# Kloudy-Sky/openintel

Measured on AMD Instinct MI355X. Metric: queries/sec + p50 latency, 10M-post/768-d hybrid BM25+cosine+RRF top-100, higher is better.
Workload: dtype f32

## Files before the change

### openintel_amd/csrc/select.hip

```cpp
#include "oi_device.h"
#include "oi_internal.h"

#define SEL_THREADS 1024
#define SEL_MAX 1024

__device__ void bitonic_sort_desc(uint64_t *a, uint32_t P) {
    const uint32_t tid = threadIdx.x;
    for (uint32_t size = 2; size <= P; size <<= 1) {
        for (uint32_t stride = size >> 1; stride > 0; stride >>= 1) {
            for (uint32_t t = tid; t < (P >> 1); t += SEL_THREADS) {
                uint32_t lo = 2 * t - (t & (stride - 1));
                uint32_t hi = lo + stride;
                bool desc = ((lo & size) == 0);
                uint64_t x = a[lo], y = a[hi];
                if ((x < y) == desc) { a[lo] = y; a[hi] = x; }
            }
            __syncthreads();
        }
    }
}

#define SEL_LDS_KEYS 8192

struct SelSource {
// ... 82 lines not shown
            if (tid < 64) {
                const uint32_t kk = s_kk;
                uint32_t mine = 0;
                for (int i = 0; i < 4; ++i) mine += hist[255 - (tid * 4 + i)];
                uint32_t incl = mine;
#pragma unroll
                for (int o = 1; o < 64; o <<= 1) {
                    uint32_t v = __shfl_up(incl, o, OI_WAVE);
                    if ((int)tid >= o) incl += v;
                }
                const unsigned long long ball = __ballot(incl >= kk);
                const uint32_t owner = ball ? (uint32_t)__builtin_ctzll(ball) : 63u;
                if (tid == owner) {
                    uint32_t cum = incl - mine;
                    int d = 255 - (int)(tid * 4);
                    for (int i = 0; i < 3; ++i, --d) {
                        const uint32_t c = hist[d];
                        if (cum + c >= kk) break;
                        cum += c;
                    }
                    s_prefix = (prefix << 8) | (uint64_t)d;
                    s_kk = kk - cum;
                    s_bin_cnt = hist[d];
                }
            }
            __syncthreads();
            if (s_bin_cnt == 1 || shift == 0) break;
        }
        const uint64_t prefix = s_prefix;
        sel_for_each(S, [&](uint64_t key) {
            if ((key >> shift) >= prefix) {
                const uint32_t pos = atomicAdd(&s_cnt, 1u);
                if (pos < SEL_MAX) sel[pos] = key;
            }
        });
        __syncthreads();
        m = s_cnt < k ? s_cnt : k;
    }
    __shared__ unsigned long long s_min;
    if (out_scores) {
        uint32_t P = 2;
        while (P < m) P <<= 1;
        for (uint32_t i = m + tid; i < P; i += SEL_THREADS) sel[i] = 0;
        __syncthreads();
        bitonic_sort_desc(sel, P);
        for (uint32_t i = tid; i < m; i += SEL_THREADS) {
            const uint64_t key = sel[i];
            out_scores[(uint64_t)q * out_stride + i] = oi_rank_key_score(key);
            out_docs[(uint64_t)q * out_stride + i] = oi_rank_key_doc(key);
        }
        if (tid == 0) { out_counts[q] = m; s_min = m ? sel[m - 1] : 0; }
    } else {
        if (tid == 0) s_min = ~0ull;
        __syncthreads();
        unsigned long long lo = ~0ull;
        for (uint32_t i = tid; i < m; i += SEL_THREADS) lo = sel[i] < lo ? sel[i] : lo;
#pragma unroll
        for (int o = 32; o > 0; o >>= 1) {
            const unsigned long long v = __shfl_xor(lo, o, OI_WAVE);
            lo = v < lo ? v : lo;
        }
        if ((tid & 63) == 0 && lo != ~0ull) atomicMin(&s_min, lo);
    }
    __syncthreads();
    if (compact) {
        for (uint32_t i = tid; i < m; i += SEL_THREADS) pool[i] = sel[i];
        for (uint32_t sg = tid; sg < n_segs; sg += SEL_THREADS) segc[sg] = 0;
        if (tid == 0) {
            carry_cnt[q] = m;
            if (m == k && tau_keys) {
                const uint32_t t = (uint32_t)(s_min >> 32);
                if (t > tau_keys[q]) tau_keys[q] = t;
            }
        }
    }
}

#define SEL_MAX_SEGS 4096
#define SEL_KPT_MAX 32
#ifdef OI_ABLATION
__device__ int sel_dbg_on;
__device__ unsigned long long sel_dbg_t[16];
#define SEL_STAMP(i) do { if (sel_dbg_on && blockIdx.x == 0 && threadIdx.x == 0) sel_dbg_t[i] = __builtin_readcyclecounter(); } while (0)
#else
#define SEL_STAMP(i) do { } while (0)
#endif
#define SEL_CAND 4096

struct SelRowMargin {
    const float *meta;
    uint32_t base;
    float qn, cq;
};
__device__ __forceinline__ float sel_row_e(const SelRowMargin *rm, uint64_t kv) {
    return rm->meta[2 * (uint64_t)(oi_rank_key_doc(kv) - rm->base) + 1];
}
__device__ __forceinline__ bool sel_row_test(const SelRowMargin *rm, uint64_t kv, float e, float edge, float eps2) {
    const float u = oi_rank_key_score(kv) + 2.002f * (e * rm->qn + rm->cq);
    return u >= edge - 9.5367431640625e-07f * (fabsf(edge) + eps2);
}
__device__ __forceinline__ bool sel_row_keep(const SelRowMargin *rm, uint64_t kv, float edge, float eps2) {
    if (!rm) return true;
    return sel_row_test(rm, kv, sel_row_e(rm, kv), edge, eps2);
}

__device__ __forceinline__ void sel_spec_words(bool have, uint32_t rth_key, float eps2, uint32_t tau, uint32_t *spec_tau, uint32_t *spec_max) {
    if (!have) { *spec_tau = tau; return; }
    const float s = oi_key_f32(rth_key) - eps2;
    const uint32_t T = s == s ? oi_f32_key(s) : 0u;
    const uint32_t st = T > tau ? T : tau;
    *spec_tau = st;
    if (st > tau && st > *spec_max) *spec_max = st;
}

struct SelShared {
    uint32_t hist[256];
    uint32_t hist2k[2048];
    uint32_t seg_off[SEL_MAX_SEGS + 1];
    uint32_t wave_tot[SEL_THREADS / 64];
    uint32_t cnt, kk, bin_cnt, n_samples;
    uint64_t prefix;
    unsigned long long min_key;
};

struct SelFlat {
    const uint64_t *pool;
    const uint32_t *seg_off;
    uint32_t n, c0, carry_cap, seg_cap, n_segs, steps;
};
struct SelCursor {
    uint32_t sg, lo, hi;
};
__device__ __forceinline__ SelCursor sel_seek(const SelFlat &K, uint32_t i) {
    const uint32_t e = i < K.c0 ? 0u : i - K.c0;
    uint32_t lo = 0, hi = K.n_segs;
    for (uint32_t s = 0; s < K.steps; ++s) {
        const uint32_t mid = (lo + hi) >> 1;
        const bool up = K.seg_off[mid] <= e;
        lo = up ? mid : lo;
        hi = up ? hi : mid;
    }
    SelCursor c;
    c.sg = lo; c.lo = K.seg_off[lo]; c.hi = K.seg_off[lo + 1];
    return c;
}
__device__ __forceinline__ uint64_t sel_at(const SelFlat &K, SelCursor &c, uint32_t i) {
    if (i < K.c0) return i;
    const uint32_t e = i - K.c0;
    while (e >= c.hi) {
        ++c.sg;
        c.lo = c.hi;
        c.hi = K.seg_off[c.sg + 1];
    }
    return (uint64_t)K.carry_cap + (uint64_t)c.sg * K.seg_cap + (e - c.lo);
}

__device__ __forceinline__ void sel_hist_add(uint32_t *hist, bool active, uint32_t digit) {
    const uint32_t lane = threadIdx.x & 63;
#pragma unroll
    for (int r = 0; r < 2; ++r) {
        const unsigned long long m = __ballot(active);
        if (!m) return;
        const uint32_t leader = (uint32_t)__builtin_ctzll(m);
        const uint32_t d0 = (uint32_t)__shfl((int)digit, (int)leader, OI_WAVE);
        const unsigned long long same = __ballot(active && digit == d0);
        if (lane == leader) atomicAdd(&hist[d0], (uint32_t)__popcll(same));
        active = active && digit != d0;
    }
    if (active) atomicAdd(&hist[digit], 1u);
}

__device__ __forceinline__ void sel_append(uint64_t *dst, uint32_t *count, uint32_t cap, bool take, uint64_t key) {
    const unsigned long long m = __ballot(take);
    if (!m) return;
    const uint32_t lane = threadIdx.x & 63, leader = (uint32_t)__builtin_ctzll(m);
    uint32_t base = 0;
    if (lane == leader) base = atomicAdd(count, (uint32_t)__popcll(m));
    base = (uint32_t)__shfl((int)base, (int)leader, OI_WAVE);
    const uint32_t pos = base + (uint32_t)__popcll(m & ((1ull << lane) - 1ull));
    if (take && pos < cap) dst[pos] = key;
}

__device__ __forceinline__ void sel_hist_add_w(uint32_t *hist, bool active, uint32_t digit, uint32_t weight) {
    const uint32_t lane = threadIdx.x & 63;
#pragma unroll
    for (int r = 0; r < 2; ++r) {
        const unsigned long long m = __ballot(active);
        if (!m) return;
        const uint32_t leader = (uint32_t)__builtin_ctzll(m);
        const uint32_t d0 = (uint32_t)__builtin_amdgcn_readlane((int)digit, (int)leader);
        const bool same = active && digit == d0;
        const uint32_t sum = (uint32_t)__builtin_amdgcn_readlane((int)oi_wave_incl_scan(same ? weight : 0u), 63);
        if (lane == leader) atomicAdd(&hist[d0], sum);
        active = active && !same;
    }
    if (active) atomicAdd(&hist[digit], weight);
}

template <class FE>
__device__ __forceinline__ void sel_threshold(FE &&for_each, uint32_t kk_in, SelShared &sh, int &shift_out, uint64_t &prefix_out) {
    const uint32_t tid = threadIdx.x;
    if (tid == 0) { sh.prefix = 0; sh.kk = kk_in; }
    int shift = 56;
    for (;; shift -= 8) {
        if (tid < 256) sh.hist[tid] = 0;
        __syncthreads();
        const uint64_t prefix = sh.prefix;
        const bool top = shift == 56;
        for_each([&](bool valid, uint64_t kv) {
            sel_hist_add(sh.hist, valid && (top || (kv >> ((shift + 8) & 63)) == prefix), (uint32_t)(kv >> shift) & 255u);
        });
        __syncthreads();
        if (tid < 64) {
            const uint32_t kk = sh.kk;
            uint32_t mine = 0;
            for (int i = 0; i < 4; ++i) mine += sh.hist[255 - (tid * 4 + i)];
            uint32_t incl = mine;
#pragma unroll
            for (int o = 1; o < 64; o <<= 1) {
                const uint32_t v = __shfl_up(incl, o, OI_WAVE);
                if ((int)tid >= o) incl += v;
            }
            const unsigned long long ball = __ballot(incl >= kk);
            const uint32_t owner = ball ? (uint32_t)__builtin_ctzll(ball) : 63u;
            if (tid == owner) {
                uint32_t cum = incl - mine;
                int d = 255 - (int)(tid * 4);
                for (int i = 0; i < 3; ++i, --d) {
                    const uint32_t c = sh.hist[d];
                    if (cum + c >= kk) break;
                    cum += c;
                }
                sh.prefix = (prefix << 8) | (uint64_t)d;
                sh.kk = kk - cum;
                sh.bin_cnt = sh.hist[d];
            }
        }
        __syncthreads();
        if (sh.bin_cnt == 1 || shift == 0) break;
    }
    shift_out = shift;
    prefix_out = sh.prefix;
    __syncthreads();
}

__device__ __forceinline__ void sel_rank_bin2k(SelShared &sh, uint32_t kk, int pass) {
    const uint32_t tid = threadIdx.x;
    {
        uint32_t v = sh.hist2k[2 * tid] + sh.hist2k[2 * tid + 1];
        v += (uint32_t)__builtin_amdgcn_update_dpp(0, (int)v, 0x111, 0xf, 0xf, false);
        v += (uint32_t)__builtin_amdgcn_update_dpp(0, (int)v, 0x112, 0xf, 0xf, false);
        v += (uint32_t)__builtin_amdgcn_update_dpp(0, (int)v, 0x114, 0xf, 0xf, false);
        v += (uint32_t)__builtin_amdgcn_update_dpp(0, (int)v, 0x118, 0xf, 0xf, false);
        if ((tid & 15u) == 15u) sh.hist[tid >> 4] = v;
    }
    __syncthreads();
    if (tid < 64) {
        const uint32_t x = sh.hist[63u - tid];
        const uint32_t incl = oi_wave_incl_scan(x);
        const unsigned long long ball = __ballot(incl >= kk);
        if (!ball) {
            if (tid == 0) sh.bin_cnt = 0xFFFFFFFFu;
        } else {
            const uint32_t l1 = (uint32_t)__builtin_ctzll(ball), sb = 63u - l1;
            const uint32_t kk2 = kk - (uint32_t)__builtin_amdgcn_readlane((int)(incl - x), (int)l1);
            const uint32_t y = tid < 32u ? sh.hist2k[32u * sb + 31u - tid] : 0u;
            const uint32_t incl2 = oi_wave_incl_scan(y);
            const unsigned long long ball2 = __ballot(incl2 >= kk2);
            const uint32_t l2 = ball2 ? (uint32_t)__builtin_ctzll(ball2) : 31u;
            const uint32_t above = (uint32_t)__builtin_amdgcn_readlane((int)(incl2 - y), (int)l2);
            if (tid == 0) {
                sh.prefix = (uint64_t)(32u * sb + 31u - l2);
                sh.kk = kk2 - above;
                sh.bin_cnt = 1u;
#ifdef OI_ABLATION
                if (sel_dbg_on > 1) {
                    uint32_t cum = 0; int dd = 2047;
                    for (; dd >= 0; --dd) { if (cum + sh.hist2k[dd] >= kk) break; cum += sh.hist2k[dd]; }
                    if ((uint32_t)dd != (uint32_t)sh.prefix || kk - cum != sh.kk)
                        printf("MISMATCH q=%u pass=%d kk=%u: walk (%d, %u) super-bin (%u, %u) sb=%u l1=%u kk2=%u l2=%u\n", blockIdx.x, pass, kk, dd, kk - cum,
                               (uint32_t)sh.prefix, sh.kk, sb, l1, kk2, l2);
                }
#endif
            }
        }
    }
    __syncthreads();
}

template <class FE>
__device__ __forceinline__ uint32_t sel_rth_score_key(FE &&for_each, uint32_t r, SelShared &sh) {
    const uint32_t tid = threadIdx.x;
    uint32_t kk = r, pfx = 0;
#pragma unroll
    for (int pass = 0; pass < 3; ++pass) {
        const int shift = pass == 0 ? 21 : pass == 1 ? 10 : 0, bits = pass == 2 ? 10 : 11;
        sh.hist2k[tid] = 0;
        sh.hist2k[tid + SEL_THREADS] = 0;
        __syncthreads();
        if (pass == 0) {
            uint32_t run_d = 0, run_c = 0;
            for_each([&](bool valid, uint64_t kv) {
                if (valid) {
                    const uint32_t d = (uint32_t)(kv >> 53);
                    if (run_c && d != run_d) { atomicAdd(&sh.hist2k[run_d], run_c); run_c = 0; }
                    run_d = d;
                    ++run_c;
                }
            });
            sel_hist_add_w(sh.hist2k, run_c != 0u, run_d, run_c);
        } else {
            for_each([&](bool valid, uint64_t kv) {
                const uint32_t sk = (uint32_t)(kv >> 32);
                if (valid && (sk >> (shift + bits)) == pfx) atomicAdd(&sh.hist2k[(sk >> shift) & ((1u << bits) - 1u)], 1u);
            });
        }
        __syncthreads();
        sel_rank_bin2k(sh, kk, 2 + pass);
        const uint32_t d = sh.bin_cnt != 0xFFFFFFFFu ? (uint32_t)sh.prefix : 0u;
        kk = sh.kk;
        __syncthreads();
        pfx = (pfx << bits) | d;
    }
    return pfx;
}

template <int KPT>
__device__ __forceinline__ uint32_t sel_flat_select(const SelFlat &K, uint32_t k, SelShared &sh, uint64_t *sel,
                                                    uint64_t *cand, float eps2, bool *in_cand, uint32_t *margin_tau,
                                                    bool *margin_overflow, const uint32_t *skip, uint32_t skip_base,
                                                    uint64_t *mc, uint32_t mcap, const SelRowMargin *rm, uint64_t *carry,
                                                    bool *in_carry, uint32_t spec_rank, uint32_t *spec_key) {
    auto skipped = [&](uint64_t kv) -> bool {
        const uint32_t d = oi_rank_key_doc(kv) - skip_base;
        return (skip[d >> 5] >> (d & 31u)) & 1u;
    };
    const uint32_t tid = threadIdx.x, lane = tid & 63, wv = tid >> 6, n = K.n;
    *in_cand = false;
    *margin_overflow = false;
    if (n == 0) return 0;
    const uint32_t kpt = (n + SEL_THREADS - 1) / SEL_THREADS;
    const uint32_t first = wv * kpt * 64 + lane, last = n - 1;
    constexpr int NR = KPT > 0 ? KPT : 1;
    uint64_t key[NR];
    uint32_t dead = 0;
    if constexpr (KPT > 0) {
        SelCursor cur = sel_seek(K, first < n ? first : last);
        uint64_t at = sel_at(K, cur, first < n ? first : last);
#pragma unroll
        for (int j = 0; j < KPT; ++j) {
            const uint32_t i = first + (uint32_t)j * 64;
            if ((uint32_t)j < kpt && i < n) at = sel_at(K, cur, i);
            key[j] = K.pool[at];
        }
        if (skip) {
#pragma unroll
            for (int j = 0; j < KPT; ++j)
                if ((uint32_t)j < kpt && first + (uint32_t)j * 64 < n && skipped(key[j])) dead |= 1u << j;
        }
    }
    auto for_each = [&](auto &&f) {
        if constexpr (KPT > 0) {
#pragma unroll
            for (int j = 0; j < KPT; ++j)
                if ((uint32_t)j < kpt) f(first + (uint32_t)j * 64 < n && !((dead >> j) & 1u), key[j]);
        } else {
            SelCursor cur = sel_seek(K, first < n ? first : last);
            uint64_t at = sel_at(K, cur, first < n ? first : last);
            for (uint32_t j0 = 0; j0 < kpt; j0 += 4) {
                uint64_t kx[4];
                bool ok[4];
#pragma unroll
                for (int u = 0; u < 4; ++u) {
                    const uint32_t i = first + (j0 + u) * 64;
                    ok[u] = j0 + u < kpt && i < n;
                    if (ok[u]) at = sel_at(K, cur, i);
                    kx[u] = K.pool[at];
                }
#pragma unroll
                for (int u = 0; u < 4; ++u) f(ok[u] && !(skip && skipped(kx[u])), kx[u]);
            }
        }
    };
    if (n <= k) {
        for_each([&](bool valid, uint64_t kv) { sel_append(sel, &sh.cnt, 2 * SEL_MAX, valid, kv); });
        __syncthreads();
        return skip ? sh.cnt : n;
    }
    SEL_STAMP(2);
    if (eps2 >= 0.f) {
        uint32_t kk = k;
        uint32_t pfx = 0;
        bool enough = true;
#pragma unroll
        for (int pass = 0; pass < 2; ++pass) {
            const int shift = 53 - 11 * pass;
            sh.hist2k[tid] = 0;
            sh.hist2k[tid + SEL_THREADS] = 0;
            __syncthreads();
            if (pass == 0) {
                uint32_t run_d = 0, run_c = 0;
                for_each([&](bool valid, uint64_t kv) {
                    if (valid) {
                        const uint32_t d = (uint32_t)(kv >> 53);
                        if (run_c && d != run_d) { atomicAdd(&sh.hist2k[run_d], run_c); run_c = 0; }
                        run_d = d;
                        ++run_c;
                    }
                });
                sel_hist_add_w(sh.hist2k, run_c != 0u, run_d, run_c);
            } else {
                for_each([&](bool valid, uint64_t kv) {
                    if (valid && (uint32_t)(kv >> 53) == pfx) atomicAdd(&sh.hist2k[(uint32_t)(kv >> shift) & 2047u], 1u);
                });
            }
            __syncthreads();
            sel_rank_bin2k(sh, kk, pass);
            enough = sh.bin_cnt != 0xFFFFFFFFu;
            const uint32_t d = (uint32_t)sh.prefix;
            kk = sh.kk;
            __syncthreads();
            if (!enough) break;
            if (pass == 0) pfx = d;
            else pfx = (pfx << 11) | d;
            SEL_STAMP(3 + pass);
        }
        if (enough) {
            uint32_t tkey = pfx << 10;
            tkey = tkey < 0x007FFFFFu ? 0x007FFFFFu : tkey;
            const uint32_t t32 = eps2 < __builtin_inff() ? oi_f32_key(oi_key_f32(tkey) - eps2) : 0u;
            uint32_t mine = 0;
            const float edge = oi_key_f32(tkey);
            auto keep = [&](bool valid, uint64_t kv) { return valid && (uint32_t)(kv >> 32) >= t32 && sel_row_keep(rm, kv, edge, eps2); };
            uint32_t verdict = 0;
            if constexpr (KPT > 0) {
#pragma unroll
                for (int j = 0; j < KPT; ++j)
                    if ((uint32_t)j < kpt && first + (uint32_t)j * 64 < n && !((dead >> j) & 1u) && (uint32_t)(key[j] >> 32) >= t32) verdict |= 1u << j;
                if (rm) {
                    constexpr int G = KPT < 8 ? KPT : 8;
#pragma unroll
                    for (int j0 = 0; j0 < KPT; j0 += G) {
                        if ((uint32_t)j0 < kpt) {
                            float e[G];
#pragma unroll
                            for (int u = 0; u < G; ++u) e[u] = (verdict >> (j0 + u)) & 1u ? sel_row_e(rm, key[j0 + u]) : 0.f;
#pragma unroll
                            for (int u = 0; u < G; ++u)
                                if (((verdict >> (j0 + u)) & 1u) && !sel_row_test(rm, key[j0 + u], e[u], edge, eps2)) verdict &= ~(1u << (j0 + u));
                        }
                    }
                }
                mine = (uint32_t)__popc(verdict);
            } else {
                for_each([&](bool valid, uint64_t kv) { mine += keep(valid, kv) ? 1u : 0u; });
            }
            const uint32_t incl = oi_wave_incl_scan(mine);
            const uint32_t tot = (uint32_t)__builtin_amdgcn_readlane((int)incl, 63);
            uint32_t base = 0;
            if (lane == 0 && tot) base = atomicAdd(&sh.cnt, tot);
            uint32_t pos = (uint32_t)__builtin_amdgcn_readfirstlane((int)base) + incl - mine;
            if constexpr (KPT > 0) {
                uint32_t stored = 0;
#pragma unroll
                for (int j = 0; j < KPT; ++j) {
                    if ((verdict >> j) & 1u) {
                        if (pos < mcap) { carry[pos] = key[j]; stored |= 1u << j; }
                        ++pos;
                    }
                }
                *in_carry = true;
                __syncthreads();
                const uint32_t c = sh.cnt, kept = c > mcap ? mcap : c;
                SEL_STAMP(5);
                if (spec_rank && kept >= spec_rank)
                    *spec_key = sel_rth_score_key([&](auto &&f) {
#pragma unroll
                        for (int j = 0; j < KPT; ++j)
                            if ((uint32_t)j < kpt) f((stored >> j) & 1u, key[j]);
                    }, spec_rank, sh);
                *in_cand = true;
                *margin_tau = t32;
                *margin_overflow = c > mcap;
                return kept;
            } else {
                for_each([&](bool valid, uint64_t kv) {
                    if (keep(valid, kv)) {
                        if (pos < mcap) mc[pos] = kv;
                        ++pos;
                    }
                });
            }
            __syncthreads();
            const uint32_t c = sh.cnt;
            *in_cand = true;
            *margin_tau = t32;
            *margin_overflow = c > mcap;
            SEL_STAMP(5);
            return c > mcap ? mcap : c;
        }
    }
    int shift;
    uint64_t prefix;
    bool selected = false;
    if (KPT != 4 && n > SEL_CAND) {
        const uint32_t js = lane % kpt, is = first + js * 64;
        bool sv = is < n;
        uint64_t sk;
        if constexpr (KPT > 0) {
            sk = key[0];
#pragma unroll
            for (int j = 1; j < KPT; ++j) sk = (uint32_t)j == js ? key[j] : sk;
            sv = sv && !((dead >> js) & 1u);
        } else {
            SelCursor cur = sel_seek(K, sv ? is : last);
            sk = K.pool[sel_at(K, cur, sv ? is : last)];
            sv = sv && !(skip && skipped(sk));
        }
        if (tid == 0) sh.n_samples = 0;
        __syncthreads();
        {
            const unsigned long long m = __ballot(sv);
            if (lane == 0 && m) atomicAdd(&sh.n_samples, (uint32_t)__popcll(m));
        }
        __syncthreads();
        const uint32_t ns = sh.n_samples;
        uint32_t r = (uint32_t)(((uint64_t)ns * (2 * k) + n - 1) / n) + 1;
        r = r > ns ? ns : r;
        sel_threshold([&](auto &&f) { f(sv, sk); }, r, sh, shift, prefix);
        for_each([&](bool valid, uint64_t kv) { sel_append(cand, &sh.cnt, SEL_CAND, valid && (kv >> shift) >= prefix, kv); });
        __syncthreads();
        const uint32_t c = sh.cnt;
        __syncthreads();
        if (tid == 0) sh.cnt = 0;
        __syncthreads();
        if (c >= k && c <= SEL_CAND) {
            uint64_t ck[SEL_CAND / SEL_THREADS];
#pragma unroll
            for (int j = 0; j < SEL_CAND / SEL_THREADS; ++j) {
                const uint32_t i = (uint32_t)j * SEL_THREADS + tid;
                ck[j] = cand[i < c ? i : c - 1];
            }
            auto cand_each = [&](auto &&f) {
#pragma unroll
                for (int j = 0; j < SEL_CAND / SEL_THREADS; ++j)
                    if ((uint32_t)j * SEL_THREADS < c) f((uint32_t)j * SEL_THREADS + tid < c, ck[j]);
            };
            if (c == k) {
                cand_each([&](bool valid, uint64_t kv) { sel_append(sel, &sh.cnt, SEL_MAX, valid, kv); });
            } else {
                sel_threshold(cand_each, k, sh, shift, prefix);
                cand_each([&](bool valid, uint64_t kv) { sel_append(sel, &sh.cnt, SEL_MAX, valid && (kv >> shift) >= prefix, kv); });
            }
            __syncthreads();
            selected = true;
        }
    }
    if (!selected) {
        sel_threshold(for_each, k, sh, shift, prefix);
        for_each([&](bool valid, uint64_t kv) { sel_append(sel, &sh.cnt, SEL_MAX, valid && (kv >> shift) >= prefix, kv); });
        __syncthreads();
    }
    const uint32_t m = sh.cnt < k ? sh.cnt : k;
    if (!(eps2 >= 0.f) || m < k) return m;
    __syncthreads();
    unsigned long long lo = ~0ull;
    for (uint32_t i = tid; i < m; i += SEL_THREADS) lo = sel[i] < lo ? sel[i] : lo;
#pragma unroll
    for (int o = 32; o > 0; o >>= 1) {
        const unsigned long long v = __shfl_xor(lo, o, OI_WAVE);
        lo = v < lo ? v : lo;
    }
    if (lane == 0 && lo != ~0ull) atomicMin(&sh.min_key, lo);
    if (tid == 0) sh.cnt = 0;
    __syncthreads();
    const uint32_t t32 = eps2 < __builtin_inff() ? oi_f32_key(oi_key_f32((uint32_t)(sh.min_key >> 32)) - eps2) : 0u;
    const float edge = oi_key_f32((uint32_t)(sh.min_key >> 32));
    for_each([&](bool valid, uint64_t kv) {
        sel_append(mc, &sh.cnt, mcap, valid && (uint32_t)(kv >> 32) >= t32 && sel_row_keep(rm, kv, edge, eps2), kv);
    });
    __syncthreads();
    const uint32_t c = sh.cnt;
    *in_cand = true;
    *margin_tau = t32;
    *margin_overflow = c > mcap;
    return c > mcap ? mcap : c;
}

__global__ __launch_bounds__(SEL_THREADS) void select_flat_kernel(
    uint64_t *pools, uint32_t *carry_cnt, uint32_t *seg_cnt, uint32_t *tau_keys, uint64_t pool_stride,
    uint32_t carry_cap, uint32_t seg_cap, uint32_t n_segs, uint32_t seg_cnt_stride, uint32_t *overflow,
    uint32_t k, int compact, float *out_scores, uint32_t *out_docs, uint32_t *out_counts, uint32_t out_stride,
    const float *eps2, uint32_t *margin_gate, const uint32_t *run_gate, const uint32_t *skip, uint32_t skip_base,
    uint64_t *cand_g, uint32_t cand_cap, const float *row_meta, uint32_t meta_base, const float *row_qn, const float *row_cq,
    uint32_t spec_rank, uint32_t *spec_tau, uint32_t *spec_max) {
    if (run_gate && *run_gate == 0u) return;
    __shared__ SelShared sh;
    __shared__ uint64_t sel[2 * SEL_MAX];
    __shared__ uint64_t cand[SEL_CAND];
    const uint32_t q = blockIdx.x, tid = threadIdx.x, lane = tid & 63, wv = tid >> 6;
    uint64_t *pool = pools + (uint64_t)q * pool_stride;
    uint32_t *segc = seg_cnt + (uint64_t)q * seg_cnt_stride;
    SEL_STAMP(0);
    const uint32_t c0_raw = carry_cnt[q];
    const float e2 = eps2 ? eps2[q] : -1.f;
    uint64_t *const mc = cand_g ? cand_g + (uint64_t)q * cand_cap : cand;
    const uint32_t mcap = cand_g ? cand_cap : SEL_CAND;
    SelRowMargin rm_v;
    if (row_meta) rm_v = SelRowMargin{row_meta, meta_base, row_qn[q], row_cq[q]};
    const SelRowMargin *rm = row_meta && e2 < __builtin_inff() ? &rm_v : nullptr;

    constexpr int SPT = SEL_MAX_SEGS / SEL_THREADS;
    uint32_t c[SPT], local = 0;
#pragma unroll
    for (int u = 0; u < SPT; ++u) {
        const uint32_t sg = tid * SPT + u;
        uint32_t v = segc[sg < n_segs ? sg : 0];
        if (sg >= n_segs) v = 0;
        if (v > seg_cap) { *overflow = 1u; v = seg_cap; }
        c[u] = v;
        local += v;
    }
    const uint32_t incl = oi_wave_incl_scan(local);
    if (lane == 63) sh.wave_tot[wv] = incl;
    if (tid == 0) { sh.cnt = 0; sh.min_key = ~0ull; }
    __syncthreads();
    uint32_t base = 0, total = 0;
#pragma unroll
    for (int w = 0; w < SEL_THREADS / 64; ++w) {
        const uint32_t t = sh.wave_tot[w];
        base += (uint32_t)w < wv ? t : 0u;
        total += t;
    }
    uint32_t run = base + incl - local;
#pragma unroll
    for (int u = 0; u < SPT; ++u) {
        const uint32_t sg = tid * SPT + u;
        if (sg < n_segs) sh.seg_off[sg] = run;
        run += c[u];
    }
    if (tid == 0) sh.seg_off[n_segs] = total;
    __syncthreads();

    SelFlat K;
    K.pool = pool; K.seg_off = sh.seg_off; K.carry_cap = carry_cap; K.seg_cap = seg_cap; K.n_segs = n_segs;
    K.c0 = c0_raw < carry_cap ? c0_raw : carry_cap;
    K.n = K.c0 + total;
    K.steps = 0;
    while ((1u << K.steps) < n_segs) ++K.steps;
    SEL_STAMP(1);

    uint32_t m, m_tau = 0;
    bool in_cand = false, m_over = false, in_carry = false;
    uint32_t spec_key = 0;
    if (K.n <= 4 * SEL_THREADS) m = sel_flat_select<4>(K, k, sh, sel, cand, e2, &in_cand, &m_tau, &m_over, skip, skip_base, mc, mcap, rm, pool, &in_carry, spec_rank, &spec_key);
    else if (K.n <= 8 * SEL_THREADS) m = sel_flat_select<8>(K, k, sh, sel, cand, e2, &in_cand, &m_tau, &m_over, skip, skip_base, mc, mcap, rm, pool, &in_carry, spec_rank, &spec_key);
    else if (K.n <= 16 * SEL_THREADS) m = sel_flat_select<16>(K, k, sh, sel, cand, e2, &in_cand, &m_tau, &m_over, skip, skip_base, mc, mcap, rm, pool, &in_carry, spec_rank, &spec_key);
    else if (K.n <= SEL_KPT_MAX * SEL_THREADS) m = sel_flat_select<SEL_KPT_MAX>(K, k, sh, sel, cand, e2, &in_cand, &m_tau, &m_over, skip, skip_base, mc, mcap, rm, pool, &in_carry, spec_rank, &spec_key);
    else m = sel_flat_select<0>(K, k, sh, sel, cand, e2, &in_cand, &m_tau, &m_over, skip, skip_base, mc, mcap, rm, pool, &in_carry, spec_rank, &spec_key);
    if (in_cand) {
        if (m_over && tid == 0 && margin_gate) *margin_gate = 1u;
        if (!in_carry)
            for (uint32_t i = tid; i < m; i += SEL_THREADS) pool[i] = mc[i];
        for (uint32_t sg = tid; sg < n_segs; sg += SEL_THREADS) segc[sg] = 0;
        if (spec_rank && !in_carry && m >= spec_rank)
            spec_key = sel_rth_score_key([&](auto &&f) {
                for (uint32_t i0 = 0; i0 < m; i0 += SEL_THREADS) f(i0 + tid < m, mc[i0 + tid < m ? i0 + tid : 0]);
            }, spec_rank, sh);
        if (tid == 0) {
            carry_cnt[q] = m;
            uint32_t tau = tau_keys ? tau_keys[q] : 0u;
            if (tau_keys && m_tau > tau) tau_keys[q] = tau = m_tau;
            if (spec_rank) sel_spec_words(m >= spec_rank, spec_key, e2, tau, spec_tau + q, spec_max + q);
        }
#ifdef OI_ABLATION
        __syncthreads();
        if (sel_dbg_on && blockIdx.x == 0 && tid == 0) {
            const unsigned long long e = __builtin_readcyclecounter();
            printf("select margin n=%u m=%u segs=%u: scan %llu, loads+skip %llu, pass0 %llu, pass1 %llu, filter %llu, compact %llu (cycles)\n", K.n, m, n_segs,
                   sel_dbg_t[1] - sel_dbg_t[0], sel_dbg_t[2] - sel_dbg_t[1], sel_dbg_t[3] - sel_dbg_t[2], sel_dbg_t[4] - sel_dbg_t[3], sel_dbg_t[5] - sel_dbg_t[4], e - sel_dbg_t[5]);
        }
#endif
        return;
    }

    if (out_scores) {
        uint32_t P = 2;
        while (P < m) P <<= 1;
        for (uint32_t i = m + tid; i < P; i += SEL_THREADS) sel[i] = 0;
        __syncthreads();
        bitonic_sort_desc(sel, P);
        for (uint32_t i = tid; i < m; i += SEL_THREADS) {
            const uint64_t key = sel[i];
            out_scores[(uint64_t)q * out_stride + i] = oi_rank_key_score(key);
            out_docs[(uint64_t)q * out_stride + i] = oi_rank_key_doc(key);
        }
        if (tid == 0) { out_counts[q] = m; sh.min_key = m ? sel[m - 1] : 0; }
    } else {
        unsigned long long lo = ~0ull;
        for (uint32_t i = tid; i < m; i += SEL_THREADS) lo = sel[i] < lo ? sel[i] : lo;
#pragma unroll
        for (int o = 32; o > 0; o >>= 1) {
            const unsigned long long v = __shfl_xor(lo, o, OI_WAVE);
            lo = v < lo ? v : lo;
        }
        if (lane == 0 && lo != ~0ull) atomicMin(&sh.min_key, lo);
    }
    __syncthreads();
    if (compact) {
        for (uint32_t i = tid; i < m; i += SEL_THREADS) pool[i] = sel[i];
        for (uint32_t sg = tid; sg < n_segs; sg += SEL_THREADS) segc[sg] = 0;
        if (tid == 0) {
            carry_cnt[q] = m;
            if (m == k && tau_keys && !eps2) {
                const uint32_t t = (uint32_t)(sh.min_key >> 32);
                if (t > tau_keys[q]) tau_keys[q] = t;
            }
        }
        if (spec_rank) {
            __syncthreads();
            if (m >= spec_rank)
                spec_key = sel_rth_score_key([&](auto &&f) {
                    for (uint32_t i0 = 0; i0 < m; i0 += SEL_THREADS) f(i0 + tid < m, sel[i0 + tid < m ? i0 + tid : 0]);
                }, spec_rank, sh);
            if (tid == 0) sel_spec_words(m >= spec_rank, spec_key, e2, tau_keys ? tau_keys[q] : 0u, spec_tau + q, spec_max + q);
        }
    }
}

int oi_launch_select(oi_ctx *ctx, const PoolView &pool, uint32_t n_queries, uint32_t k, bool compact,
                     float *out_scores, uint32_t *out_docs, uint32_t *out_counts, uint32_t out_stride,
                     const SelectExtra *extra) {
    if (n_queries == 0) return OI_OK;
    OI_REQUIRE(k >= 1 && k <= OI_MAX_DEPTH && k <= pool.carry_cap, "select: k=%u outside [1,%u]", k, OI_MAX_DEPTH);
    ProfScope ps(ctx, "select");
    static const bool v1 = oi_ablation_env("OI_SELECT_V1") != nullptr;
#ifdef OI_ABLATION
    static const bool stamps = [] {
        const int on = oi_ablation_env("OI_SELECT_STAMPS") ? std::max(1, atoi(oi_ablation_env("OI_SELECT_STAMPS"))) : 0;
        (void)hipMemcpyToSymbol(HIP_SYMBOL(sel_dbg_on), &on, sizeof(int));
        return on != 0;
    }();
    (void)stamps;
#endif
    const bool special = extra && (extra->eps2 || extra->run_gate);
    if (special) {
        OI_REQUIRE(pool.n_segs <= SEL_MAX_SEGS, "select: %u segments (margin / gated selects take <= %u)", pool.n_segs, SEL_MAX_SEGS);
        const uint32_t mcap = extra->cand ? extra->cand_cap : SEL_CAND;
        OI_REQUIRE(!extra->eps2 || (compact && !out_scores && pool.carry_cap >= mcap),
                   "select: margin mode compacts into a carry region of >= %u keys", mcap);
    }
    const bool spec = extra && extra->spec_rank;
    OI_REQUIRE(!spec || (extra->eps2 && extra->spec_tau && extra->spec_max && pool.tau_keys),
               "select: a speculative threshold needs margin mode, thresholds and both output arrays");
    if ((!v1 || special) && pool.n_segs <= SEL_MAX_SEGS) {
        hipLaunchKernelGGL(select_flat_kernel, dim3(n_queries), dim3(SEL_THREADS), 0, ctx->stream, pool.keys,
                           pool.carry_cnt, pool.seg_cnt, pool.tau_keys, pool.stride, pool.carry_cap, pool.seg_cap,
                           pool.n_segs, pool.seg_cnt_stride, pool.overflow, k, compact ? 1 : 0, out_scores, out_docs,
                           out_counts, out_stride, extra ? extra->eps2 : nullptr, extra ? extra->margin_gate : nullptr,
                           extra ? extra->run_gate : nullptr, extra && extra->eps2 ? extra->skip_bitmap : nullptr,
                           extra ? extra->skip_base : 0u, extra && extra->eps2 ? extra->cand : nullptr,
                           extra && extra->eps2 ? extra->cand_cap : 0u, extra && extra->eps2 ? extra->row_meta : nullptr,
                           extra ? extra->meta_base : 0u, extra ? extra->row_qn : nullptr, extra ? extra->row_cq : nullptr,
                           spec ? extra->spec_rank : 0u, spec ? extra->spec_tau : nullptr, spec ? extra->spec_max : nullptr);
        OI_HIP_CHECK(hipGetLastError());
        return OI_OK;
    }
    hipLaunchKernelGGL(select_topk_kernel, dim3(n_queries), dim3(SEL_THREADS), 0, ctx->stream, pool.keys,
                       pool.carry_cnt, pool.seg_cnt, pool.tau_keys, pool.stride, pool.carry_cap, pool.seg_cap,
                       pool.n_segs, pool.seg_cnt_stride, pool.overflow, k, compact ? 1 : 0, out_scores, out_docs,
                       out_counts, out_stride);
    OI_HIP_CHECK(hipGetLastError());
    return OI_OK;
}

__global__ void lists_to_pool_kernel(const float *scores, const uint32_t *docs, const uint32_t *counts,
                                     uint64_t shard_stride, uint64_t count_stride, uint32_t n_queries,
                                     uint32_t depth, uint64_t *pools, uint32_t *carry_cnt,
                                     uint32_t *seg_cnt, uint64_t pool_stride, uint32_t carry_cap,
                                     uint32_t seg_cnt_stride) {
    const uint32_t q = blockIdx.x, sh = blockIdx.y;
    uint32_t c = counts[(uint64_t)sh * count_stride + q];
    if (c > depth) c = depth;
    const uint64_t src = (uint64_t)sh * shard_stride + (uint64_t)q * depth;
    uint64_t *seg = pools + (uint64_t)q * pool_stride + carry_cap + (uint64_t)sh * depth;
    for (uint32_t i = threadIdx.x; i < c; i += blockDim.x) seg[i] = oi_rank_key(scores[src + i], docs[src + i]);
    if (threadIdx.x == 0) {
        seg_cnt[(uint64_t)q * seg_cnt_stride + sh] = c;
        if (sh == 0) carry_cnt[q] = 0;
    }
}

int oi_launch_lists_to_pool(oi_ctx *ctx, const float *scores, const uint32_t *docs,
                            const uint32_t *counts, uint64_t shard_stride, uint64_t count_stride,
                            uint32_t n_shards, uint32_t n_queries, uint32_t depth, const PoolView &pool) {
    if (n_queries == 0) return OI_OK;
    OI_REQUIRE(pool.seg_cap == depth && pool.n_segs == n_shards, "merge: pool geometry mismatch");
    hipLaunchKernelGGL(lists_to_pool_kernel, dim3(n_queries, n_shards), dim3(256), 0, ctx->stream, scores, docs,
                       counts, shard_stride, count_stride, n_queries, depth, pool.keys, pool.carry_cnt, pool.seg_cnt, pool.stride,
                       pool.carry_cap, pool.seg_cnt_stride);
    OI_HIP_CHECK(hipGetLastError());
    return OI_OK;
}

#define RRF_HASH 4096
__global__ __launch_bounds__(SEL_THREADS) void rrf_kernel(const uint32_t *docs_a, const uint32_t *counts_a,
                                                          const uint32_t *docs_b, const uint32_t *counts_b,
                                                          uint32_t depth, uint32_t k, float *scores_out,
                                                          uint32_t *docs_out, uint32_t *counts_out) {
    __shared__ uint32_t h_doc[RRF_HASH];
    __shared__ uint32_t h_idx[RRF_HASH];
    __shared__ uint32_t a_match[SEL_MAX];
    __shared__ uint64_t u[2 * SEL_MAX];
    __shared__ uint32_t s_extra;

    const uint32_t q = blockIdx.x, tid = threadIdx.x;
    uint32_t na = counts_a[q], nb = counts_b[q];
    if (na > depth) na = depth;
    if (nb > depth) nb = depth;
    const uint32_t *da = docs_a + (uint64_t)q * depth, *db = docs_b + (uint64_t)q * depth;

    for (uint32_t i = tid; i < RRF_HASH; i += SEL_THREADS) h_idx[i] = 0;
    for (uint32_t i = tid; i < SEL_MAX; i += SEL_THREADS) a_match[i] = 0;
    if (tid == 0) s_extra = 0;
    __syncthreads();
    for (uint32_t i = tid; i < na; i += SEL_THREADS) {
        uint32_t d = da[i];
        uint32_t h = (d * 2654435761u) >> 20;
        for (;;) {
            uint32_t prev = atomicCAS(&h_idx[h], 0u, i + 1);
            if (prev == 0) { h_doc[h] = d; break; }
            h = (h + 1) & (RRF_HASH - 1);
        }
    }
    __syncthreads();
    for (uint32_t j = tid; j < nb; j += SEL_THREADS) {
        uint32_t d = db[j];
        uint32_t h = (d * 2654435761u) >> 20;
        uint32_t hit = 0;
        for (;;) {
            uint32_t ix = h_idx[h];
            if (ix == 0) break;
            if (h_doc[h] == d) { hit = ix; break; }
            h = (h + 1) & (RRF_HASH - 1);
        }
        if (hit) a_match[hit - 1] = j + 1;
        else {
            uint32_t pos = atomicAdd(&s_extra, 1u);
            float c = 1.0f / (60.0f + (float)(j + 1));
            u[na + pos] = oi_rank_key(c, d);
        }
    }
    __syncthreads();
    for (uint32_t i = tid; i < na; i += SEL_THREADS) {
        float s = 1.0f / (60.0f + (float)(i + 1));
        uint32_t j1 = a_match[i];
        if (j1) s = s + 1.0f / (60.0f + (float)j1);
        u[i] = oi_rank_key(s, da[i]);
    }
    __syncthreads();
    const uint32_t m = na + s_extra;
    uint32_t P = 2;
    while (P < m) P <<= 1;
    for (uint32_t i = m + tid; i < P; i += SEL_THREADS) u[i] = 0;
    __syncthreads();
    bitonic_sort_desc(u, P);
    const uint32_t out = m < k ? m : k;
    for (uint32_t i = tid; i < out; i += SEL_THREADS) {
        scores_out[(uint64_t)q * k + i] = oi_rank_key_score(u[i]);
        docs_out[(uint64_t)q * k + i] = oi_rank_key_doc(u[i]);
    }
    if (tid == 0) counts_out[q] = out;
}

int oi_launch_rrf(oi_ctx *ctx, const uint32_t *docs_a, const uint32_t *counts_a, const uint32_t *docs_b,
                  const uint32_t *counts_b, uint32_t n_queries, uint32_t depth, uint32_t k,
                  float *scores_out, uint32_t *docs_out, uint32_t *counts_out) {
    if (n_queries == 0) return OI_OK;
    OI_REQUIRE(depth >= 1 && depth <= OI_MAX_DEPTH, "rrf: depth=%u outside [1,%u]", depth, OI_MAX_DEPTH);
    OI_REQUIRE(k >= 1 && k <= OI_MAX_DEPTH, "rrf: k=%u outside [1,%u]", k, OI_MAX_DEPTH);
    ProfScope ps(ctx, "rrf");
    hipLaunchKernelGGL(rrf_kernel, dim3(n_queries), dim3(SEL_THREADS), 0, ctx->stream, docs_a, counts_a,
                       docs_b, counts_b, depth, k, scores_out, docs_out, counts_out);
    OI_HIP_CHECK(hipGetLastError());
    return OI_OK;
}
```

Before: 36730.

## Prune RRF candidates by rank bound and select top-k via rank counting

The RRF fusion kernel now computes a rank reach bound from k and discards entries whose fused score cannot reach the k-th place. When enough entries survive within the bound, it skips the bitonic sort and places each survivor by counting how many keys exceed it, using vectorised LDS reads. It also assigns one thread per list entry with preloaded doc ids instead of strided loops. This removes the log^2 sort barriers for the common case, at the cost of an O(m) scan per thread and reliance on the correctness of the pruning bound.

After: 37040 (median of 6 runs). About the same (+0.9%).

```diff
diff --git a/openintel_amd/csrc/select.hip b/openintel_amd/csrc/select.hip
--- a/openintel_amd/csrc/select.hip
+++ b/openintel_amd/csrc/select.hip
@@ -910,6 +910,14 @@
 }
 
 #define RRF_HASH 4096
+#define RRF_RANK_MAX 1024
+__device__ __forceinline__ float rrf_c(uint32_t rank) { return 1.0f / (60.0f + (float)rank); }
+__device__ __forceinline__ uint32_t rrf_reach(uint32_t k) {
+    const float L = rrf_c(k);
+    uint32_t R = 2 * k + 58;
+    while (!(2.0f * rrf_c(R + 1) < L)) ++R;
+    return R;
+}
 __global__ __launch_bounds__(SEL_THREADS) void rrf_kernel(const uint32_t *docs_a, const uint32_t *counts_a,
                                                           const uint32_t *docs_b, const uint32_t *counts_b,
                                                           uint32_t depth, uint32_t k, float *scores_out,
@@ -917,31 +925,34 @@
     __shared__ uint32_t h_doc[RRF_HASH];
     __shared__ uint32_t h_idx[RRF_HASH];
     __shared__ uint32_t a_match[SEL_MAX];
-    __shared__ uint64_t u[2 * SEL_MAX];
-    __shared__ uint32_t s_extra;
-
+    __shared__ __attribute__((aligned(16))) uint64_t u[2 * SEL_MAX];
+    __shared__ uint32_t s_cnt;
+
+    static_assert(SEL_THREADS >= SEL_MAX, "one thread per list entry");
     const uint32_t q = blockIdx.x, tid = threadIdx.x;
+    const uint32_t my_a = tid < depth ? docs_a[(uint64_t)q * depth + tid] : 0u, my_b = tid < depth ? docs_b[(uint64_t)q * depth + tid] : 0u;
     uint32_t na = counts_a[q], nb = counts_b[q];
     if (na > depth) na = depth;
     if (nb > depth) nb = depth;
-    const uint32_t *da = docs_a + (uint64_t)q * depth, *db = docs_b + (uint64_t)q * depth;
+    const bool bounded = na >= k || nb >= k;
+    const uint32_t R = bounded ? rrf_reach(k) : 0xffffffffu;
+    const float L = bounded ? rrf_c(k) : 0.f;
 
     for (uint32_t i = tid; i < RRF_HASH; i += SEL_THREADS) h_idx[i] = 0;
     for (uint32_t i = tid; i < SEL_MAX; i += SEL_THREADS) a_match[i] = 0;
-    if (tid == 0) s_extra = 0;
-    __syncthreads();
-    for (uint32_t i = tid; i < na; i += SEL_THREADS) {
-        uint32_t d = da[i];
-        uint32_t h = (d * 2654435761u) >> 20;
+    if (tid == 0) s_cnt = 0;
+    __syncthreads();
+    if (tid < na) {
+        uint32_t h = (my_a * 2654435761u) >> 20;
         for (;;) {
-            uint32_t prev = atomicCAS(&h_idx[h], 0u, i + 1);
-            if (prev == 0) { h_doc[h] = d; break; }
+            uint32_t prev = atomicCAS(&h_idx[h], 0u, tid + 1);
+            if (prev == 0) { h_doc[h] = my_a; break; }
             h = (h + 1) & (RRF_HASH - 1);
         }
     }
     __syncthreads();
-    for (uint32_t j = tid; j < nb; j += SEL_THREADS) {
-        uint32_t d = db[j];
+    if (tid < nb) {
+        const uint32_t j = tid, d = my_b;
         uint32_t h = (d * 2654435761u) >> 20;
         uint32_t hit = 0;
         for (;;) {
@@ -951,32 +962,49 @@
             h = (h + 1) & (RRF_HASH - 1);
         }
         if (hit) a_match[hit - 1] = j + 1;
-        else {
-            uint32_t pos = atomicAdd(&s_extra, 1u);
-            float c = 1.0f / (60.0f + (float)(j + 1));
-            u[na + pos] = oi_rank_key(c, d);
-        }
-    }
-    __syncthreads();
-    for (uint32_t i = tid; i < na; i += SEL_THREADS) {
-        float s = 1.0f / (60.0f + (float)(i + 1));
-        uint32_t j1 = a_match[i];
-        if (j1) s = s + 1.0f / (60.0f + (float)j1);
-        u[i] = oi_rank_key(s, da[i]);
-    }
-    __syncthreads();
-    const uint32_t m = na + s_extra;
+        else if (j + 1 <= R && rrf_c(j + 1) >= L) u[atomicAdd(&s_cnt, 1u)] = oi_rank_key(rrf_c(j + 1), d);
+    }
+    __syncthreads();
+    if (tid < na) {
+        const uint32_t j1 = a_match[tid];
+        if (tid + 1 <= R || (j1 != 0 && j1 <= R)) {
+            float s = rrf_c(tid + 1);
+            if (j1) s = s + rrf_c(j1);
+            if (s >= L) u[atomicAdd(&s_cnt, 1u)] = oi_rank_key(s, my_a);
+        }
+    }
+    __syncthreads();
+    const uint32_t m = s_cnt;
+    const uint32_t out = m < k ? m : k;
+    if (tid == 0) counts_out[q] = out;
+    if (bounded && m <= RRF_RANK_MAX) {
+        if (tid == 0) u[m] = 0;
+        __syncthreads();
+        if (tid < m) {
+            const uint64_t mine = u[tid];
+            const ulonglong2 *u2 = reinterpret_cast<const ulonglong2 *>(u);
+            uint32_t above = 0;
+#pragma unroll 4
+            for (uint32_t j = 0; j < (m + 1) / 2; ++j) {
+                const ulonglong2 v = u2[j];
+                above += (v.x > mine ? 1u : 0u) + (v.y > mine ? 1u : 0u);
+            }
+            if (above < k) {
+                scores_out[(uint64_t)q * k + above] = oi_rank_key_score(mine);
+                docs_out[(uint64_t)q * k + above] = oi_rank_key_doc(mine);
+            }
+        }
+        return;
+    }
     uint32_t P = 2;
     while (P < m) P <<= 1;
     for (uint32_t i = m + tid; i < P; i += SEL_THREADS) u[i] = 0;
     __syncthreads();
     bitonic_sort_desc(u, P);
-    const uint32_t out = m < k ? m : k;
     for (uint32_t i = tid; i < out; i += SEL_THREADS) {
         scores_out[(uint64_t)q * k + i] = oi_rank_key_score(u[i]);
         docs_out[(uint64_t)q * k + i] = oi_rank_key_doc(u[i]);
     }
-    if (tid == 0) counts_out[q] = out;
 }
 
 int oi_launch_rrf(oi_ctx *ctx, const uint32_t *docs_a, const uint32_t *counts_a, const uint32_t *docs_b,
```

## Reuse pass-0 histogram for speculative threshold and prefetch row margins early

Applied to the files above, without the earlier changes.

Keeps the first radix pass histogram in its own shared buffer so the speculative rank-threshold computation can skip rebuilding it when no edge keys were dropped. Row-margin metadata is gathered right after key loads, for small keys-per-thread, so its latency overlaps the histogram passes. Segment counts are loaded in a separate loop before clamping. The cost is 8KB more LDS per block, extra registers for the early margin values, and an edge_lost check to keep the reuse correct.

Measured after the change: 36710 before, 37010 after (median of 6 runs). About the same (+0.8%).

```diff
diff --git a/openintel_amd/csrc/select.hip b/openintel_amd/csrc/select.hip
--- a/openintel_amd/csrc/select.hip
+++ b/openintel_amd/csrc/select.hip
@@ -188,8 +188,12 @@
 __device__ int sel_dbg_on;
 __device__ unsigned long long sel_dbg_t[16];
 #define SEL_STAMP(i) do { if (sel_dbg_on && blockIdx.x == 0 && threadIdx.x == 0) sel_dbg_t[i] = __builtin_readcyclecounter(); } while (0)
+#define SEL_N_STAMPS 11
+__device__ int sel_off;
+#define SEL_ON(bit) (!(sel_off & (bit)))
 #else
 #define SEL_STAMP(i) do { } while (0)
+#define SEL_ON(bit) true
 #endif
 #define SEL_CAND 4096
 
@@ -201,6 +205,10 @@
 __device__ __forceinline__ float sel_row_e(const SelRowMargin *rm, uint64_t kv) {
     return rm->meta[2 * (uint64_t)(oi_rank_key_doc(kv) - rm->base) + 1];
 }
+__device__ __forceinline__ float sel_row_e_if(const SelRowMargin *rm, uint64_t kv, bool on) {
+    const uint32_t r = on ? oi_rank_key_doc(kv) - rm->base : 0u;
+    return rm->meta[2 * (uint64_t)r + 1];
+}
 __device__ __forceinline__ bool sel_row_test(const SelRowMargin *rm, uint64_t kv, float e, float edge, float eps2) {
     const float u = oi_rank_key_score(kv) + 2.002f * (e * rm->qn + rm->cq);
     return u >= edge - 9.5367431640625e-07f * (fabsf(edge) + eps2);
@@ -224,7 +232,7 @@
     uint32_t hist2k[2048];
     uint32_t seg_off[SEL_MAX_SEGS + 1];
     uint32_t wave_tot[SEL_THREADS / 64];
-    uint32_t cnt, kk, bin_cnt, n_samples;
+    uint32_t cnt, kk, bin_cnt, n_samples, edge_lost;
     uint64_t prefix;
     unsigned long long min_key;
 };
@@ -350,10 +358,10 @@
     __syncthreads();
 }
 
-__device__ __forceinline__ void sel_rank_bin2k(SelShared &sh, uint32_t kk, int pass) {
+__device__ __forceinline__ void sel_rank_bin2k(SelShared &sh, const uint32_t *h2k, uint32_t kk, int pass) {
     const uint32_t tid = threadIdx.x;
     {
-        uint32_t v = sh.hist2k[2 * tid] + sh.hist2k[2 * tid + 1];
+        uint32_t v = h2k[2 * tid] + h2k[2 * tid + 1];
         v += (uint32_t)__builtin_amdgcn_update_dpp(0, (int)v, 0x111, 0xf, 0xf, false);
         v += (uint32_t)__builtin_amdgcn_update_dpp(0, (int)v, 0x112, 0xf, 0xf, false);
         v += (uint32_t)__builtin_amdgcn_update_dpp(0, (int)v, 0x114, 0xf, 0xf, false);
@@ -370,7 +378,7 @@
         } else {
             const uint32_t l1 = (uint32_t)__builtin_ctzll(ball), sb = 63u - l1;
             const uint32_t kk2 = kk - (uint32_t)__builtin_amdgcn_readlane((int)(incl - x), (int)l1);
-            const uint32_t y = tid < 32u ? sh.hist2k[32u * sb + 31u - tid] : 0u;
+            const uint32_t y = tid < 32u ? h2k[32u * sb + 31u - tid] : 0u;
             const uint32_t incl2 = oi_wave_incl_scan(y);
             const unsigned long long ball2 = __ballot(incl2 >= kk2);
             const uint32_t l2 = ball2 ? (uint32_t)__builtin_ctzll(ball2) : 31u;
@@ -382,7 +390,7 @@
 #ifdef OI_ABLATION
                 if (sel_dbg_on > 1) {
                     uint32_t cum = 0; int dd = 2047;
-                    for (; dd >= 0; --dd) { if (cum + sh.hist2k[dd] >= kk) break; cum += sh.hist2k[dd]; }
+                    for (; dd >= 0; --dd) { if (cum + h2k[dd] >= kk) break; cum += h2k[dd]; }
                     if ((uint32_t)dd != (uint32_t)sh.prefix || kk - cum != sh.kk)
                         printf("MISMATCH q=%u pass=%d kk=%u: walk (%d, %u) super-bin (%u, %u) sb=%u l1=%u kk2=%u l2=%u\n", blockIdx.x, pass, kk, dd, kk - cum,
                                (uint32_t)sh.prefix, sh.kk, sb, l1, kk2, l2);
@@ -395,12 +403,20 @@
 }
 
 template <class FE>
-__device__ __forceinline__ uint32_t sel_rth_score_key(FE &&for_each, uint32_t r, SelShared &sh) {
+__device__ __forceinline__ uint32_t sel_rth_score_key(FE &&for_each, uint32_t r, SelShared &sh, const uint32_t *hist0 = nullptr) {
     const uint32_t tid = threadIdx.x;
     uint32_t kk = r, pfx = 0;
 #pragma unroll
     for (int pass = 0; pass < 3; ++pass) {
         const int shift = pass == 0 ? 21 : pass == 1 ? 10 : 0, bits = pass == 2 ? 10 : 11;
+        if (pass == 0 && hist0) {
+            sel_rank_bin2k(sh, hist0, kk, 2);
+            pfx = sh.bin_cnt != 0xFFFFFFFFu ? (uint32_t)sh.prefix : 0u;
+            kk = sh.kk;
+            __syncthreads();
+            SEL_STAMP(8);
+            continue;
+        }
         sh.hist2k[tid] = 0;
         sh.hist2k[tid + SEL_THREADS] = 0;
         __syncthreads();
@@ -422,11 +438,12 @@
             });
         }
         __syncthreads();
-        sel_rank_bin2k(sh, kk, 2 + pass);
+        sel_rank_bin2k(sh, sh.hist2k, kk, 2 + pass);
         const uint32_t d = sh.bin_cnt != 0xFFFFFFFFu ? (uint32_t)sh.prefix : 0u;
         kk = sh.kk;
         __syncthreads();
         pfx = (pfx << bits) | d;
+        SEL_STAMP(8 + pass);
     }
     return pfx;
 }
@@ -436,7 +453,7 @@
                                                     uint64_t *cand, float eps2, bool *in_cand, uint32_t *margin_tau,
                                                     bool *margin_overflow, const uint32_t *skip, uint32_t skip_base,
                                                     uint64_t *mc, uint32_t mcap, const SelRowMargin *rm, uint64_t *carry,
-                                                    bool *in_carry, uint32_t spec_rank, uint32_t *spec_key) {
+                                                    bool *in_carry, uint32_t spec_rank, uint32_t *spec_key, uint32_t *hist0) {
     auto skipped = [&](uint64_t kv) -> bool {
         const uint32_t d = oi_rank_key_doc(kv) - skip_base;
         return (skip[d >> 5] >> (d & 31u)) & 1u;
@@ -450,6 +467,9 @@
     constexpr int NR = KPT > 0 ? KPT : 1;
     uint64_t key[NR];
     uint32_t dead = 0;
+    constexpr bool EARLY_E = KPT > 0 && KPT <= 16;
+    float er[EARLY_E ? KPT : 1];
+    const bool early_e = EARLY_E && rm && eps2 >= 0.f && n > k && SEL_ON(2);
     if constexpr (KPT > 0) {
         SelCursor cur = sel_seek(K, first < n ? first : last);
         uint64_t at = sel_at(K, cur, first < n ? first : last);
@@ -463,6 +483,16 @@
 #pragma unroll
             for (int j = 0; j < KPT; ++j)
                 if ((uint32_t)j < kpt && first + (uint32_t)j * 64 < n && skipped(key[j])) dead |= 1u << j;
+        }
+        if constexpr (EARLY_E) {
+            if (early_e) {
+#pragma unroll
+                for (int j = 0; j < KPT; ++j)
+                    er[j] = sel_row_e_if(rm, key[j], (uint32_t)j < kpt && first + (uint32_t)j * 64 < n && !((dead >> j) & 1u));
+            } else {
+#pragma unroll
+                for (int j = 0; j < KPT; ++j) er[j] = 0.f;
+            }
         }
     }
     auto for_each = [&](auto &&f) {
@@ -501,27 +531,29 @@
 #pragma unroll
         for (int pass = 0; pass < 2; ++pass) {
             const int shift = 53 - 11 * pass;
-            sh.hist2k[tid] = 0;
-            sh.hist2k[tid + SEL_THREADS] = 0;
+            uint32_t *const h2k = pass == 0 ? hist0 : sh.hist2k;
+            h2k[tid] = 0;
+            h2k[tid + SEL_THREADS] = 0;
+            if (pass == 0 && tid == 0) sh.edge_lost = 0;
             __syncthreads();
             if (pass == 0) {
                 uint32_t run_d = 0, run_c = 0;
                 for_each([&](bool valid, uint64_t kv) {
                     if (valid) {
                         const uint32_t d = (uint32_t)(kv >> 53);
-                        if (run_c && d != run_d) { atomicAdd(&sh.hist2k[run_d], run_c); run_c = 0; }
+                        if (run_c && d != run_d) { atomicAdd(&h2k[run_d], run_c); run_c = 0; }
                         run_d = d;
                         ++run_c;
                     }
                 });
-                sel_hist_add_w(sh.hist2k, run_c != 0u, run_d, run_c);
+                sel_hist_add_w(h2k, run_c != 0u, run_d, run_c);
             } else {
                 for_each([&](bool valid, uint64_t kv) {
-                    if (valid && (uint32_t)(kv >> 53) == pfx) atomicAdd(&sh.hist2k[(uint32_t)(kv >> shift) & 2047u], 1u);
+                    if (valid && (uint32_t)(kv >> 53) == pfx) atomicAdd(&h2k[(uint32_t)(kv >> shift) & 2047u], 1u);
                 });
             }
             __syncthreads();
-            sel_rank_bin2k(sh, kk, pass);
+            sel_rank_bin2k(sh, h2k, kk, pass);
             enough = sh.bin_cnt != 0xFFFFFFFFu;
             const uint32_t d = (uint32_t)sh.prefix;
             kk = sh.kk;
@@ -543,14 +575,21 @@
 #pragma unroll
                 for (int j = 0; j < KPT; ++j)
                     if ((uint32_t)j < kpt && first + (uint32_t)j * 64 < n && !((dead >> j) & 1u) && (uint32_t)(key[j] >> 32) >= t32) verdict |= 1u << j;
-                if (rm) {
+                SEL_STAMP(5);
+                if (EARLY_E && early_e) {
+                    if constexpr (EARLY_E) {
+#pragma unroll
+                        for (int j = 0; j < KPT; ++j)
+                            if (((verdict >> j) & 1u) && !sel_row_test(rm, key[j], er[j], edge, eps2)) verdict &= ~(1u << j);
+                    }
+                } else if (rm) {
                     constexpr int G = KPT < 8 ? KPT : 8;
 #pragma unroll
                     for (int j0 = 0; j0 < KPT; j0 += G) {
                         if ((uint32_t)j0 < kpt) {
                             float e[G];
 #pragma unroll
-                            for (int u = 0; u < G; ++u) e[u] = (verdict >> (j0 + u)) & 1u ? sel_row_e(rm, key[j0 + u]) : 0.f;
+                            for (int u = 0; u < G; ++u) e[u] = sel_row_e_if(rm, key[j0 + u], (verdict >> (j0 + u)) & 1u);
 #pragma unroll
                             for (int u = 0; u < G; ++u)
                                 if (((verdict >> (j0 + u)) & 1u) && !sel_row_test(rm, key[j0 + u], e[u], edge, eps2)) verdict &= ~(1u << (j0 + u));
@@ -558,6 +597,7 @@
                     }
                 }
                 mine = (uint32_t)__popc(verdict);
+                SEL_STAMP(6);
             } else {
                 for_each([&](bool valid, uint64_t kv) { mine += keep(valid, kv) ? 1u : 0u; });
             }
@@ -576,15 +616,22 @@
                     }
                 }
                 *in_carry = true;
+                if (spec_rank) {
+                    uint32_t at_edge = 0;
+#pragma unroll
+                    for (int j = 0; j < KPT; ++j)
+                        if ((uint32_t)j < kpt && first + (uint32_t)j * 64 < n && !((dead >> j) & 1u) && (uint32_t)(key[j] >> 32) >= (pfx << 10)) at_edge |= 1u << j;
+                    if (at_edge & ~stored) sh.edge_lost = 1u;
+                }
                 __syncthreads();
                 const uint32_t c = sh.cnt, kept = c > mcap ? mcap : c;
-                SEL_STAMP(5);
+                SEL_STAMP(7);
                 if (spec_rank && kept >= spec_rank)
                     *spec_key = sel_rth_score_key([&](auto &&f) {
 #pragma unroll
                         for (int j = 0; j < KPT; ++j)
                             if ((uint32_t)j < kpt) f((stored >> j) & 1u, key[j]);
-                    }, spec_rank, sh);
+                    }, spec_rank, sh, spec_rank <= k && !sh.edge_lost && SEL_ON(4) ? hist0 : nullptr);
                 *in_cand = true;
                 *margin_tau = t32;
                 *margin_overflow = c > mcap;
@@ -602,7 +649,7 @@
             *in_cand = true;
             *margin_tau = t32;
             *margin_overflow = c > mcap;
-            SEL_STAMP(5);
+            SEL_STAMP(7);
             return c > mcap ? mcap : c;
         }
     }
@@ -704,9 +751,14 @@
     __shared__ SelShared sh;
     __shared__ uint64_t sel[2 * SEL_MAX];
     __shared__ uint64_t cand[SEL_CAND];
+    __shared__ uint32_t hist0[2048];
     const uint32_t q = blockIdx.x, tid = threadIdx.x, lane = tid & 63, wv = tid >> 6;
     uint64_t *pool = pools + (uint64_t)q * pool_stride;
     uint32_t *segc = seg_cnt + (uint64_t)q * seg_cnt_stride;
+#ifdef OI_ABLATION
+    if (sel_dbg_on && blockIdx.x == 0 && threadIdx.x == 0)
+        for (int i = 0; i < 16; ++i) sel_dbg_t[i] = 0;
+#endif
     SEL_STAMP(0);
     const uint32_t c0_raw = carry_cnt[q];
     const float e2 = eps2 ? eps2[q] : -1.f;
@@ -719,9 +771,11 @@
     constexpr int SPT = SEL_MAX_SEGS / SEL_THREADS;
     uint32_t c[SPT], local = 0;
 #pragma unroll
+    for (int u = 0; u < SPT; ++u) c[u] = segc[tid * SPT + u < n_segs ? tid * SPT + u : 0];
+#pragma unroll
     for (int u = 0; u < SPT; ++u) {
         const uint32_t sg = tid * SPT + u;
-        uint32_t v = segc[sg < n_segs ? sg : 0];
+        uint32_t v = c[u];
         if (sg >= n_segs) v = 0;
         if (v > seg_cap) { *overflow = 1u; v = seg_cap; }
         c[u] = v;
@@ -759,11 +813,11 @@
     uint32_t m, m_tau = 0;
     bool in_cand = false, m_over = false, in_carry = false;
     uint32_t spec_key = 0;
-    if (K.n <= 4 * SEL_THREADS) m = sel_flat_select<4>(K, k, sh, sel, cand, e2, &in_cand, &m_tau, &m_over, skip, skip_base, mc, mcap, rm, pool, &in_carry, spec_rank, &spec_key);
-    else if (K.n <= 8 * SEL_THREADS) m = sel_flat_select<8>(K, k, sh, sel, cand, e2, &in_cand, &m_tau, &m_over, skip, skip_base, mc, mcap, rm, pool, &in_carry, spec_rank, &spec_key);
-    else if (K.n <= 16 * SEL_THREADS) m = sel_flat_select<16>(K, k, sh, sel, cand, e2, &in_cand, &m_tau, &m_over, skip, skip_base, mc, mcap, rm, pool, &in_carry, spec_rank, &spec_key);
-    else if (K.n <= SEL_KPT_MAX * SEL_THREADS) m = sel_flat_select<SEL_KPT_MAX>(K, k, sh, sel, cand, e2, &in_cand, &m_tau, &m_over, skip, skip_base, mc, mcap, rm, pool, &in_carry, spec_rank, &spec_key);
-    else m = sel_flat_select<0>(K, k, sh, sel, cand, e2, &in_cand, &m_tau, &m_over, skip, skip_base, mc, mcap, rm, pool, &in_carry, spec_rank, &spec_key);
+    if (K.n <= 4 * SEL_THREADS) m = sel_flat_select<4>(K, k, sh, sel, cand, e2, &in_cand, &m_tau, &m_over, skip, skip_base, mc, mcap, rm, pool, &in_carry, spec_rank, &spec_key, hist0);
+    else if (K.n <= 8 * SEL_THREADS) m = sel_flat_select<8>(K, k, sh, sel, cand, e2, &in_cand, &m_tau, &m_over, skip, skip_base, mc, mcap, rm, pool, &in_carry, spec_rank, &spec_key, hist0);
+    else if (K.n <= 16 * SEL_THREADS) m = sel_flat_select<16>(K, k, sh, sel, cand, e2, &in_cand, &m_tau, &m_over, skip, skip_base, mc, mcap, rm, pool, &in_carry, spec_rank, &spec_key, hist0);
+    else if (K.n <= SEL_KPT_MAX * SEL_THREADS) m = sel_flat_select<SEL_KPT_MAX>(K, k, sh, sel, cand, e2, &in_cand, &m_tau, &m_over, skip, skip_base, mc, mcap, rm, pool, &in_carry, spec_rank, &spec_key, hist0);
+    else m = sel_flat_select<0>(K, k, sh, sel, cand, e2, &in_cand, &m_tau, &m_over, skip, skip_base, mc, mcap, rm, pool, &in_carry, spec_rank, &spec_key, hist0);
     if (in_cand) {
         if (m_over && tid == 0 && margin_gate) *margin_gate = 1u;
         if (!in_carry)
@@ -783,8 +837,14 @@
         __syncthreads();
         if (sel_dbg_on && blockIdx.x == 0 && tid == 0) {
             const unsigned long long e = __builtin_readcyclecounter();
-            printf("select margin n=%u m=%u segs=%u: scan %llu, loads+skip %llu, pass0 %llu, pass1 %llu, filter %llu, compact %llu (cycles)\n", K.n, m, n_segs,
-                   sel_dbg_t[1] - sel_dbg_t[0], sel_dbg_t[2] - sel_dbg_t[1], sel_dbg_t[3] - sel_dbg_t[2], sel_dbg_t[4] - sel_dbg_t[3], sel_dbg_t[5] - sel_dbg_t[4], e - sel_dbg_t[5]);
+            unsigned long long prev = sel_dbg_t[0], d[SEL_N_STAMPS];
+            for (int i = 1; i < SEL_N_STAMPS; ++i) {
+                d[i] = sel_dbg_t[i] ? sel_dbg_t[i] - prev : 0ull;
+                prev = sel_dbg_t[i] ? sel_dbg_t[i] : prev;
+            }
+            printf("select margin n=%u c0=%u m=%u segs=%u rm=%d spec=%u: segment scan %llu, seek + key loads %llu, pass 0 %llu, pass 1 %llu, global test %llu, "
+                   "gather + row test %llu, scan + store %llu, prediction 0 %llu, prediction 1 %llu, prediction 2 %llu, epilogue %llu, all %llu (cycles)\n",
+                   K.n, K.c0, m, n_segs, rm ? 1 : 0, spec_rank, d[1], d[2], d[3], d[4], d[5], d[6], d[7], d[8], d[9], d[10], e - prev, e - sel_dbg_t[0]);
         }
 #endif
         return;
@@ -845,6 +905,8 @@
     static const bool stamps = [] {
         const int on = oi_ablation_env("OI_SELECT_STAMPS") ? std::max(1, atoi(oi_ablation_env("OI_SELECT_STAMPS"))) : 0;
         (void)hipMemcpyToSymbol(HIP_SYMBOL(sel_dbg_on), &on, sizeof(int));
+        const int off = oi_ablation_env("OI_SELECT_OFF") ? atoi(oi_ablation_env("OI_SELECT_OFF")) : 0;
+        (void)hipMemcpyToSymbol(HIP_SYMBOL(sel_off), &off, sizeof(int));
         return on != 0;
     }();
     (void)stamps;
```
